# mapillary/OpenSfM

Measured on AMD Instinct MI355X. Metric: image-pairs matched/sec (+ BA LM-iters/sec, 5k cams / 500k pts), higher is better.
Workload: dtype i8 (exact int32 accumulate) + f64 RANSAC

## Files before the change

### opensfm_amd/csrc/ba.hip

```cpp
#ifdef OSFM_HIPEMU
#include <cassert>
#endif
#include <chrono>
#include <cmath>
#include <cstdio>
#include <cstring>
#include <numeric>
#include <vector>

#include <rocprim/rocprim.hpp>

#include "ba_math.h"
#include "osfm_internal.h"

using namespace osfm_ba;

namespace {

constexpr int kCoopObs = 256;

typedef double osfm_v2d __attribute__((ext_vector_type(2)));
__device__ __forceinline__ void st2(double *p, double a, double b) {
  osfm_v2d v;
  v.x = a;
// ... 3248 lines not shown
  for (int t = threadIdx.x; t < n; t += blockDim.x) v[0] += Bc[(long)i * n + t] * z[t];
  block_sum<1, 1024>(v, lds);
  if (threadIdx.x == 0) y[i] = r[cam0 + i] - v[0];
}
__global__ void border_rhs_apply_kernel(const double *SigInv, const double *y, double *z, int nb, int cam0) {
  const int i = blockIdx.x * blockDim.x + threadIdx.x;
  if (i >= nb) return;
  double acc = 0.0;
  for (int j = 0; j < nb; j++) acc += SigInv[i * nb + j] * y[j];
  z[cam0 + i] = acc;
}
__global__ void border_update_kernel(const double *W, double *z, int nb, int n, int cam0) {
  const int t = blockIdx.x * blockDim.x + threadIdx.x;
  if (t >= n) return;
  double acc = 0.0;
  for (int j = 0; j < nb; j++) acc += W[(long)j * n + t] * z[cam0 + j];
  z[t] -= acc;
}


__global__ void border_sigma_kernel(const double *Cm, const double *dots, double *SigInv, int nb, int *status) {
  if (threadIdx.x != 0 || blockIdx.x != 0) return;
  double Sg[36], Inv[36];
  for (int i = 0; i < nb * nb; i++) {
    Sg[i] = Cm[i] - dots[i];
    Inv[i] = 0.0;
  }
  for (int i = 0; i < nb; i++) Inv[i * nb + i] = 1.0;
  int bad = 0;
  for (int c = 0; c < nb && !bad; c++) {
    int piv = c;
    for (int r2 = c + 1; r2 < nb; r2++)
      if (fabs(Sg[r2 * nb + c]) > fabs(Sg[piv * nb + c])) piv = r2;
    const double pv = Sg[piv * nb + c];
    if (!(fabs(pv) > 0) || !(fabs(pv) < 1.0 / 0.0)) { bad = 1; break; }
    for (int q = 0; q < nb; q++) {
      const double t0 = Sg[c * nb + q], t1 = Inv[c * nb + q];
      Sg[c * nb + q] = Sg[piv * nb + q];
      Sg[piv * nb + q] = t0;
      Inv[c * nb + q] = Inv[piv * nb + q];
      Inv[piv * nb + q] = t1;
    }
    const double ip = 1.0 / Sg[c * nb + c];
    for (int q = 0; q < nb; q++) { Sg[c * nb + q] *= ip; Inv[c * nb + q] *= ip; }
    for (int r2 = 0; r2 < nb; r2++) {
      if (r2 == c) continue;
      const double f = Sg[r2 * nb + c];
      for (int q = 0; q < nb; q++) { Sg[r2 * nb + q] -= f * Sg[c * nb + q]; Inv[r2 * nb + q] -= f * Inv[c * nb + q]; }
    }
  }
  *status = bad;
  for (int i = 0; i < nb * nb; i++) SigInv[i] = bad ? 0.0 : Inv[i];
}
template <int NB>
__global__ void __launch_bounds__(kCoopObs) border_point_kernel(Dev d, double *wB) {
  constexpr int NC_ = NB / 3;
  __shared__ double gsum[kCoopObs * 9];
  __shared__ int gcam[kCoopObs];
  __shared__ double vpt[kCoopObs * 3 * NB];
  const int tid = threadIdx.x;
  const int p0 = d.wg_pt[blockIdx.x], p1 = d.wg_pt[blockIdx.x + 1];
  const long o0 = d.pt_off[p0], o1 = d.pt_off[p1];
  const int nobs = (int)(o1 - o0);
  if (nobs <= kCoopObs) {
    double t0[3] = {0, 0, 0}, t1[3] = {0, 0, 0}, jp[6] = {0, 0, 0, 0, 0, 0};
    int pl = 0, cam = 0;
    const long o = o0 + tid;
    if (tid < nobs) {
      pl = d.o_point[o] - p0;
      const int so = d.o_shot[o];
      cam = d.shot_camera[so];
      const double *sck = d.sc_red + d.cam0 + 3 * cam;
      double jk[6];
      row_jk(d, o, so, jk);
#pragma unroll
      for (int k = 0; k < 3; k++) {
        t0[k] = jk[k] * sck[k];
        t1[k] = jk[3 + k] * sck[k];
      }
#pragma unroll
      for (int j = 0; j < 6; j++) jp[j] = JA(o, R_JP + j);
#pragma unroll
      for (int k = 0; k < 3; k++)
#pragma unroll
        for (int j = 0; j < 3; j++) gsum[9 * tid + 3 * k + j] = jp[j] * t0[k] + jp[3 + j] * t1[k];
      gcam[tid] = cam;
    }
    __syncthreads();
    if (tid < p1 - p0) {
      const int p = p0 + tid;
      double u[NB][3];
#pragma unroll
      for (int c = 0; c < NB; c++) u[c][0] = u[c][1] = u[c][2] = 0.0;
      const int a = (int)(d.pt_off[p] - o0), b = (int)(d.pt_off[p + 1] - o0);
      for (int k = a; k < b; k++) {
        const int cc = gcam[k];
#pragma unroll
        for (int c = 0; c < NC_; c++)
          if (c == cc)
#pragma unroll
            for (int q = 0; q < 3; q++)
#pragma unroll
              for (int j = 0; j < 3; j++) u[3 * c + q][j] += gsum[9 * k + 3 * q + j];
      }
      const double *Hh = d.Hhat + 6 * (long)p;
#pragma unroll
      for (int c = 0; c < NB; c++) {
        vpt[(3 * tid + 0) * NB + c] = Hh[0] * u[c][0] + Hh[1] * u[c][1] + Hh[2] * u[c][2];
        vpt[(3 * tid + 1) * NB + c] = Hh[1] * u[c][0] + Hh[3] * u[c][1] + Hh[4] * u[c][2];
        vpt[(3 * tid + 2) * NB + c] = Hh[2] * u[c][0] + Hh[4] * u[c][1] + Hh[5] * u[c][2];
      }
    }
    __syncthreads();
    if (tid < nobs) {
      double2 *dst = reinterpret_cast<double2 *>(wB + 2L * NB * o);
#pragma unroll
      for (int c = 0; c < NB; c++) {
        const double v0 = vpt[(3 * pl + 0) * NB + c], v1 = vpt[(3 * pl + 1) * NB + c], v2 = vpt[(3 * pl + 2) * NB + c];
        const bool own = (c / 3) == cam;
        st2(reinterpret_cast<double *>(dst + c), (own ? t0[c % 3] : 0.0) - (jp[0] * v0 + jp[1] * v1 + jp[2] * v2),
                      (own ? t1[c % 3] : 0.0) - (jp[3] * v0 + jp[4] * v1 + jp[5] * v2));
      }
    }
    return;
  }
  double u[NB][3];
#pragma unroll
  for (int c = 0; c < NB; c++) u[c][0] = u[c][1] = u[c][2] = 0.0;
  for (long o = o0 + tid; o < o1; o += kCoopObs) {
    const int so = d.o_shot[o], cam = d.shot_camera[so];
    const double *sck = d.sc_red + d.cam0 + 3 * cam;
    double jk[6];
    row_jk(d, o, so, jk);
#pragma unroll
    for (int c = 0; c < NC_; c++)
      if (c == cam)
#pragma unroll
        for (int k = 0; k < 3; k++) {
          const double t0 = jk[k] * sck[k], t1 = jk[3 + k] * sck[k];
#pragma unroll
          for (int j = 0; j < 3; j++) u[3 * c + k][j] += JA(o, R_JP + j) * t0 + JA(o, R_JP + 3 + j) * t1;
        }
  }
#pragma unroll
  for (int c = 0; c < NB; c++)
#pragma unroll
    for (int j = 0; j < 3; j++) vpt[(3 * tid + j) * NB + c] = u[c][j];
  __syncthreads();
  for (int h = kCoopObs / 2; h >= 1; h >>= 1) {
    if (tid < h)
      for (int q = 0; q < 3 * NB; q++) vpt[3 * NB * tid + q] += vpt[3 * NB * (tid + h) + q];
    __syncthreads();
  }
  const double *Hh = d.Hhat + 6 * (long)p0;
  double v[NB][3];
#pragma unroll
  for (int c = 0; c < NB; c++) {
    const double u0 = vpt[0 * NB + c], u1 = vpt[1 * NB + c], u2 = vpt[2 * NB + c];
    v[c][0] = Hh[0] * u0 + Hh[1] * u1 + Hh[2] * u2;
    v[c][1] = Hh[1] * u0 + Hh[3] * u1 + Hh[4] * u2;
    v[c][2] = Hh[2] * u0 + Hh[4] * u1 + Hh[5] * u2;
  }
  for (long o = o0 + tid; o < o1; o += kCoopObs) {
    const int so = d.o_shot[o], cam = d.shot_camera[so];
    const double *sck = d.sc_red + d.cam0 + 3 * cam;
    double jk[6];
    row_jk(d, o, so, jk);
#pragma unroll
    for (int c = 0; c < NB; c++) {
      const bool own = (c / 3) == cam;
      const double t0 = own ? jk[c % 3] * sck[c % 3] : 0.0, t1 = own ? jk[3 + c % 3] * sck[c % 3] : 0.0;
      wB[(2L * NB * o) + 2 * c] = t0 - (JA(o, R_JP) * v[c][0] + JA(o, R_JP + 1) * v[c][1] + JA(o, R_JP + 2) * v[c][2]);
      wB[(2L * NB * o) + 2 * c + 1] = t1 - (JA(o, R_JP + 3) * v[c][0] + JA(o, R_JP + 4) * v[c][1] + JA(o, R_JP + 5) * v[c][2]);
    }
  }
}

template <int NB, int W>
__global__ void __launch_bounds__(64 * W) border_shot_kernel(Dev d, const double *wB, double *Bc, double *partB) {
  __shared__ double red[W > 1 ? W * 9 : 1];
  const int s = (int)xcd_contiguous(blockIdx.x, gridDim.x), lane = threadIdx.x;
  double v[NB][9];
#pragma unroll
  for (int c = 0; c < NB; c++)
#pragma unroll
    for (int i = 0; i < 9; i++) v[c][i] = 0.0;
  const ShotFrame f = shot_frame(d, s);
  for (long k = d.shot_off[s] + lane; k < d.shot_off[s + 1]; k += 64 * W) {
    const long o = d.shot_obs[k];
    const double2 *src = reinterpret_cast<const double2 *>(wB + 2L * NB * o);
    double jc0[6], jc1[6], jk0[3], jk1[3];
    {
      double rr[2], jp[6], jc[12], jk[6];
      sm_row(d, f, k, d.sm_wt[k], rr, jp, jc, jk);
#pragma unroll
      for (int j = 0; j < 6; j++) {
        jc0[j] = jc[j];
        jc1[j] = jc[6 + j];
      }
#pragma unroll
      for (int j = 0; j < 3; j++) {
        jk0[j] = jk[j];
        jk1[j] = jk[3 + j];
      }
    }
#pragma unroll
    for (int c = 0; c < NB; c++) {
      const double2 wv = src[c];
#pragma unroll
      for (int j = 0; j < 6; j++) v[c][j] += jc0[j] * wv.x + jc1[j] * wv.y;
#pragma unroll
      for (int j = 0; j < 3; j++) v[c][6 + j] += jk0[j] * wv.x + jk1[j] * wv.y;
    }
  }
#pragma unroll
  for (int c = 0; c < NB; c++) {
    shot_sum<9, W>(v[c], red);
    if (W > 1) __syncthreads();
  }
  if (lane == 0) {
    const long n6 = 6L * d.S;
#pragma unroll
    for (int c = 0; c < NB; c++) {
      for (int j = 0; j < 6; j++) Bc[c * n6 + 6 * s + j] = d.sc_red[6 * s + j] * v[c][j];
      for (int j = 0; j < 3; j++) partB[(long)s * 3 * NB + 3 * c + j] = v[c][6 + j];
    }
  }
}

template <int NB>
__global__ void __launch_bounds__(TPB) border_cam_kernel(Dev d, const double *partB, double *Cm, double radius) {
  __shared__ double lds[4 * 3 * NB];
  const int cam = blockIdx.x;
  double v[3 * NB];
#pragma unroll
  for (int i = 0; i < 3 * NB; i++) v[i] = 0.0;
  for (int s = threadIdx.x; s < d.S; s += TPB)
    if (d.shot_camera[s] == cam)
#pragma unroll
      for (int i = 0; i < 3 * NB; i++) v[i] += partB[(long)s * 3 * NB + i];
  block_sum<3 * NB, TPB>(v, lds);
  if (threadIdx.x == 0)
    for (int c = 0; c < NB; c++)
      for (int k = 0; k < 3; k++) {
        const int i = d.cam0 + 3 * cam + k;
        const bool diag = (3 * cam + k) == c;
        const double y = diag ? d.sc_red[i] : 0.0;
        Cm[(3 * cam + k) * NB + c] = d.sc_red[i] * (v[3 * c + k] + d.prior_diag[i] * y) + (diag ? d.D_red[i] / radius : 0.0);
      }
}

__global__ void iota_int_kernel(int *a, long n) {
  const long i = (long)blockIdx.x * TPB + threadIdx.x;
  if (i < n) a[i] = (int)i;
}
__global__ void gather_byte_kernel(const int *idx, const unsigned char *src, long n, unsigned char *dst) {
  const long i = (long)blockIdx.x * TPB + threadIdx.x;
  if (i < n) dst[i] = src[idx[i]];
}
__global__ void gen_shot_off_kernel(const long *view_off, const int *inst_view0, int S, long *shot_off) {
  const int i = blockIdx.x * TPB + threadIdx.x;
  if (i <= S) shot_off[i] = view_off[inst_view0[i]];
}
__global__ void gather_int_kernel(const int *idx, const int *src, long n, int *dst) {
  const long i = (long)blockIdx.x * TPB + threadIdx.x;
  if (i < n) dst[i] = src[idx[i]];
}
__global__ void lower_bound_kernel(const int *sorted, long n, int nv, long *off) {
  const long v = (long)blockIdx.x * TPB + threadIdx.x;
  if (v > nv) return;
  long lo = 0, hi = n;
  while (lo < hi) {
    const long mid = (lo + hi) >> 1;
    if (sorted[mid] < (int)v)
      lo = mid + 1;
    else
      hi = mid;
  }
  off[v] = lo;
}
// ... 258 lines not shown
      if (e != hipSuccess && want > bytes) {
        (void)hipGetLastError();
        e = ctx ? b->alloc(ctx, bytes) : b->alloc(bytes);
      }
      if (e != hipSuccess) {
        b->p = nullptr;
        delete b;
        return nullptr;
      }
#ifdef OSFM_HIPEMU
      memset(b->p, 0xFF, b->bytes);
#endif
      slabs.push_back(b);
      cur = (char *)b->p;
      left = b->bytes;
      next_slab = std::min(next_slab * 2, (size_t)2 << 30);
    }
    T *p = (T *)cur;
    cur += bytes;
    left -= bytes;
    return p;
  }
  hipStream_t st = nullptr;
  size_t staged = 0;
  static constexpr size_t kStageBytes = (size_t)4 << 20, kStageMax = (size_t)256 << 10;
  template <typename T>
  T *upload(const T *h, size_t n, hipError_t &e) {
    T *p = alloc<T>(n, e);
    if (e != hipSuccess || n == 0) return p;
    const size_t bytes = n * sizeof(T), padded = (bytes + 63) / 64 * 64;
    if (ctx && st && bytes <= kStageMax && staged + padded <= kStageBytes) {
      if (!ctx->h_stage && hipHostMalloc(&ctx->h_stage, kStageBytes, hipHostMallocDefault) != hipSuccess) {
        ctx->h_stage = nullptr;
        (void)hipGetLastError();
      }
      if (ctx->h_stage) {
        char *dst = (char *)ctx->h_stage + staged;
        memcpy(dst, h, bytes);
        staged += padded;
        e = hipMemcpyAsync(p, dst, bytes, hipMemcpyHostToDevice, st);
        return p;
      }
    }
    e = hipMemcpy(p, h, bytes, hipMemcpyHostToDevice);
    return p;
  }
};

inline int nblk(long n, int t = TPB) { return (int)std::max<long>(1, (n + t - 1) / t); }

struct BaSwitches {
  bool no_sband = getenv("OSFM_BA_NO_SBAND") != nullptr;
  bool check_band = getenv("OSFM_BA_CHECK_BAND") != nullptr;
  bool band_per_shot = getenv("OSFM_BA_BAND_PER_SHOT") != nullptr;
  bool wide_ldlt = getenv("OSFM_BA_WIDE_LDLT") != nullptr;
  const char *dense_cr_budget = getenv("OSFM_BA_DENSE_CR_BUDGET");
  bool gen_full_rows = getenv("OSFM_BA_GEN_FULL_ROWS") != nullptr;
  bool no_fast = getenv("OSFM_BA_NO_FAST") != nullptr;
  int fast_fail_at = getenv("OSFM_BA_FAST_FAIL_AT") ? atoi(getenv("OSFM_BA_FAST_FAIL_AT")) : -1;
  bool trace = getenv("OSFM_BA_TRACE") != nullptr;
  bool spin = getenv("OSFM_BA_NO_SPIN") == nullptr;
  double spin_us = getenv("OSFM_BA_SPIN_US") ? atof(getenv("OSFM_BA_SPIN_US")) : 2000.0;
};

int ba_kernel_attributes(int device) {
  static OsfmPerDeviceOnce once;
  return once.run(device, []() -> int {
    constexpr int kWholeLds = 160 * 1024;
    const auto max_lds = [](const void *kernel, int bytes) { return hipFuncSetAttribute(kernel, hipFuncAttributeMaxDynamicSharedMemorySize, bytes); };
    OSFM_HIP(max_lds((const void *)band_assemble_kernel, kWholeLds));
    OSFM_HIP(max_lds((const void *)band_assemble_compact_kernel, kWholeLds));
    OSFM_HIP(max_lds((const void *)band_mfma_kernel<1>, 96 * 1024));
    OSFM_HIP(max_lds((const void *)band_mfma_kernel<2>, 96 * 1024));
    OSFM_HIP(max_lds((const void *)band_mfma_kernel<3>, 96 * 1024));
    OSFM_HIP(max_lds((const void *)band_mfma_kernel<4>, 96 * 1024));
    OSFM_HIP(max_lds((const void *)band_mfma_kernel<5>, 96 * 1024));
    OSFM_HIP(max_lds((const void *)band_mfma_kernel<6>, 96 * 1024));
    for (int q = 2; q <= 10; q++) OSFM_HIP(max_lds((const void *)bcr_level_for(q).fn, kWholeLds));
    OSFM_HIP(max_lds((const void *)sband_factor_kernel, kWholeLds - 256));
    OSFM_HIP(max_lds((const void *)sband_solve_kernel, kWholeLds));
    OSFM_HIP(max_lds((const void *)wide_factor_kernel, kWholeLds));
    OSFM_HIP(max_lds((const void *)dgj_pivot_kernel, kWholeLds));
    OSFM_HIP(max_lds((const void *)band_cholesky_kernel, kWholeLds));
    OSFM_HIP(max_lds((const void *)ctri_inverse_kernel, kWholeLds));
    OSFM_HIP(max_lds((const void *)gen_border_sigma_kernel, kWholeLds - 256));
    return OSFM_OK;
  });
}

typedef void (*band_mfma_fn)(Dev);
inline band_mfma_fn band_mfma_for(int nt) {
  static constexpr band_mfma_fn fn[6] = {band_mfma_kernel<1>, band_mfma_kernel<2>, band_mfma_kernel<3>, band_mfma_kernel<4>, band_mfma_kernel<5>, band_mfma_kernel<6>};
  return fn[nt >= 1 && nt <= 5 ? nt - 1 : 5];
}

struct SolvePlan {
  int nbord = 0;
  int bw_true = 0;
  int track_repeats_shot = 0;
  int *bp_keys = nullptr, *bp_pts = nullptr;
  bool border_ok = true;
  bool all_cams_fixed = false;
  bool wide = false;
  bool dense_cr = false;
  bool win_band = false;
  int win_grid = 0;
// ... 28 lines not shown
  const double rho = cost_change / model_change;
  if (O->verbose & 1)
    fprintf(stderr, "[osfm_ba] it %d cost %.9e -> %.9e rho %.3f radius %.3e pcg %d\n", iter, cost, cost_n, rho, radius, pcg_iterations);
  if (rho > 1e-3) {
    const double t = 2.0 * rho - 1.0;
    radius = radius / std::fmax(1.0 / 3.0, 1.0 - t * t * t);
    radius = std::fmin(1e16, radius);
    decrease_factor = 2.0;
    return LmVerdict::Accepted;
  }
  radius = radius / decrease_factor;
  decrease_factor *= 2.0;
  return LmVerdict::Rejected;
}

struct Solver {
  osfm_ctx *ctx;
  Dev d;
  BaSwitches sw;
  hipStream_t st;
  int loss;
  double loss_a;
  hipStream_t st2 = nullptr;
  hipEvent_t ev_fork = nullptr, ev_join = nullptr;
  int *d_perm = nullptr;
  int *d_status = nullptr;
  double *d_reproj = nullptr;
  double *hscal = nullptr;
  int *hstat = nullptr;
  double *hrr = nullptr;
  int *hseq = nullptr;
  int seq = 0, nbr_ = 0;
  bool spin = false;
  double spin_us = 0.0;
  void *dev_pinned = nullptr;
  int *g_cols = nullptr, *g_col_pos = nullptr;
  int g_ncols = 0;
  double *g_wB = nullptr, *g_vpartB = nullptr;
  int gen_uniform_model = -1;
  bool gen_compact = false;
  bool have_bpri = false;
  std::vector<unsigned char> gen_col_slot;
  bool use_band = false, use_ctri = false, use_bcr = false, use_border = false, use_wide = false;
  bool use_sband = false;
  bool sband_solved = false;
  bool z_solved = false;
  bool joined = true;
  bool have_scale = false;
  double cur_radius = 0.0;
  bool cams_inert = false;
  double *Bc = nullptr, *Wb = nullptr, *SigInv = nullptr, *dots = nullptr;
  double *yb = nullptr;
  static constexpr int kBorderRhsSplit = 6 * 512;
  double *wB = nullptr, *partB = nullptr, *dCm = nullptr;
  double *sbL = nullptr;

  int pinned(int nbr) {
    const size_t need = (size_t)(32 + 2 + nbr + 8) * sizeof(double);
    if (ctx->h_pinned_bytes < need) {
      if (ctx->h_pinned) (void)hipHostFree(ctx->h_pinned);
      ctx->h_pinned = nullptr;
      ctx->h_pinned_bytes = 0;
      OSFM_HIP(hipHostMalloc(&ctx->h_pinned, std::max<size_t>(need, 65536), hipHostMallocDefault));
      ctx->h_pinned_bytes = std::max<size_t>(need, 65536);
    }
    hscal = (double *)ctx->h_pinned;
    hstat = (int *)(hscal + 32);
    hrr = hscal + 34;
    hseq = (int *)(hscal + 34 + nbr);
    nbr_ = nbr;
    for (int i = 0; i < 34; i++) hscal[i] = 0.0;
    *hseq = 0;
    seq = 0;
    spin = sw.spin;
    spin_us = sw.spin_us;
    if (spin) OSFM_HIP(hipHostGetDevicePointer(&dev_pinned, ctx->h_pinned, 0));
    return OSFM_OK;
  }
  int fetch(const double *a, int na, int ha_off, const int *b = nullptr, int nb = 0, int hb_off = 0, const double *c = nullptr, int nc = 0) {
    if (!spin) {
      if (na) OSFM_HIP(hipMemcpyAsync(hscal + ha_off, a, (size_t)na * sizeof(double), hipMemcpyDeviceToHost, st));
      if (nb) OSFM_HIP(hipMemcpyAsync(hstat + hb_off, b, (size_t)nb * sizeof(int), hipMemcpyDeviceToHost, st));
      if (nc) OSFM_HIP(hipMemcpyAsync(hrr, c, (size_t)nc * sizeof(double), hipMemcpyDeviceToHost, st));
      OSFM_HIP(hipStreamSynchronize(st));
      return OSFM_OK;
    }
    double *dh = (double *)dev_pinned;
    const int want = ++seq;
    hipLaunchKernelGGL(publish_kernel, dim3(1), dim3(64), 0, st, a, na, dh + ha_off, b, nb, (int *)(dh + 32) + hb_off, c, nc, dh + 34, (int *)(dh + 34 + nbr_), want);
    OSFM_HIP(hipGetLastError());
    const auto t0 = std::chrono::steady_clock::now();
    for (long it = 0; __atomic_load_n(hseq, __ATOMIC_ACQUIRE) != want; it++) {
      if ((it & 0x3FF) == 0x3FF && std::chrono::duration<double>(std::chrono::steady_clock::now() - t0).count() * 1e6 > spin_us) {
        OSFM_HIP(hipStreamSynchronize(st));
        OSFM_REQUIRE(__atomic_load_n(hseq, __ATOMIC_ACQUIRE) == want, OSFM_E_HIP, "the device never published round trip %d", want);
      }
    }
    return OSFM_OK;
  }

  void rot(const double *poses) { hipLaunchKernelGGL(shot_rot_kernel, dim3(nblk(d.S, 64)), dim3(64), 0, st, d, poses); }

  template <class F>
  void with_gen_model(F &&f) const {
    using std::integral_constant;
    if (d.g.NRr == 3) f(integral_constant<int, 3>{}, integral_constant<int, -1>{});
// ... 352 lines not shown
  void rhs_enqueue(double radius, hipStream_t sq) {
    if (d.gen) {
      gen_rows_apply(1, sq);
      hipLaunchKernelGGL(gen_schur_finish_kernel, dim3(nbr_), dim3(TPB), 0, sq, d, (const double *)d.x, (const double *)d.y, d.b, radius, 1, d.M > 0 ? 1 : 0, 0, (double *)nullptr);
    } else {
      hipLaunchKernelGGL(schur_point_coop_kernel<1>, dim3(d.nwg), dim3(kCoopObs), 0, sq, d, d.y);
      schur_shot(sq);
      hipLaunchKernelGGL(schur_finish_kernel, dim3(matvec_parts()), dim3(TPB), 0, sq, d, (const double *)d.x, (const double *)d.y, d.b, radius, 1, cams_inert ? 1 : 0,
                         (double *)nullptr);
    }
  }
  int fork_side(hipStream_t side2) {
    OSFM_HIP(hipEventRecord(ev_fork, st));
    OSFM_HIP(hipStreamWaitEvent(side2, ev_fork, 0));
    return OSFM_OK;
  }
  int join() {
    if (!joined) OSFM_HIP(hipStreamWaitEvent(st, ev_join, 0));
    joined = true;
    return OSFM_OK;
  }
  int check_band(const SolvePlan &pl, double radius) {
    const size_t nbd = (size_t)d.S * (d.bw + 1) * 36;
    std::vector<double> b_win(nbd), b_shot(nbd);
    OSFM_HIP(hipMemcpyAsync(b_win.data(), d.band, nbd * sizeof(double), hipMemcpyDeviceToHost, st));
    hipLaunchKernelGGL(band_assemble_kernel, dim3(d.S), dim3(TPB), (size_t)(d.bw + 1) * 36 * pl.band_copies * sizeof(double), st, d, radius, pl.band_copies, 0, d.bw + 1);
    OSFM_HIP(hipMemcpyAsync(b_shot.data(), d.band, nbd * sizeof(double), hipMemcpyDeviceToHost, st));
    OSFM_HIP(hipStreamSynchronize(st));
    double amax = 0, dmax = 0;
    for (size_t q = 0; q < nbd; q++) {
      amax = std::max(amax, std::fabs(b_shot[q]));
      dmax = std::max(dmax, std::fabs(b_shot[q] - b_win[q]));
    }
    OSFM_REQUIRE(dmax <= 1e-10 * amax, OSFM_E_NUMERIC, "band_mfma_kernel differs from band_assemble_kernel: max |diff| %.3e against max |entry| %.3e", dmax, amax);
    OSFM_HIP(hipMemcpyAsync(d.band, b_win.data(), nbd * sizeof(double), hipMemcpyHostToDevice, st));
    OSFM_HIP(hipStreamSynchronize(st));
    return OSFM_OK;
  }
  int assemble_band(const SolvePlan &pl, double radius) {
    if (pl.win_band) {
      hipLaunchKernelGGL(band_mfma_for(d.bpNT), dim3(pl.win_grid), dim3(384), pl.win_lds, st, d);
      hipLaunchKernelGGL(band_finish_kernel, dim3(nblk((long)d.S * (d.bw + 1) * 36)), dim3(TPB), 0, st, d, radius);
      if (sw.check_band) OSFM_TRY(check_band(pl, radius));
    } else if (d.bslot) {
      hipLaunchKernelGGL(band_assemble_compact_kernel, dim3(d.S), dim3(TPB), (size_t)pl.bslot_n * 36 * pl.bslot_copies * sizeof(double) + ((d.bw + 1 + 15) / 16) * 16, st, d,
                         radius, pl.bslot_copies, pl.bslot_n);
    } else {
      for (int lo = 0; lo <= d.bw; lo += pl.band_slice)
        hipLaunchKernelGGL(band_assemble_kernel, dim3(d.S), dim3(TPB), (size_t)std::min(pl.band_slice, d.bw + 1 - lo) * 36 * pl.band_copies * sizeof(double), st, d,
                           radius, pl.band_copies, lo, std::min(pl.band_slice, d.bw + 1 - lo));
    }
    return OSFM_OK;
  }
  int side_work(const SolvePlan &pl, double radius, bool fork_here) {
    const hipStream_t sx = pl.side2 ? pl.side2 : st;
    if (pl.side2 && fork_here) OSFM_TRY(fork_side(pl.side2));
    if (pl.want_border && d.gen) {
      gen_border_columns(radius, sx);
    } else if (pl.want_border) {
      if (3 * d.NC == 3) {
        hipLaunchKernelGGL(border_point_kernel<3>, dim3(d.nwg), dim3(kCoopObs), 0, sx, d, wB);
        if (shot_waves() > 1) hipLaunchKernelGGL((border_shot_kernel<3, kShotWavesSmall>), dim3(d.S), dim3(64 * kShotWavesSmall), 0, sx, d, wB, Bc, partB);
        else hipLaunchKernelGGL((border_shot_kernel<3, 1>), dim3(d.S), dim3(64), 0, sx, d, wB, Bc, partB);
        hipLaunchKernelGGL(border_cam_kernel<3>, dim3(d.NC), dim3(TPB), 0, sx, d, partB, dCm, radius);
      } else {
        hipLaunchKernelGGL(border_point_kernel<6>, dim3(d.nwg), dim3(kCoopObs), 0, sx, d, wB);
        if (shot_waves() > 1) hipLaunchKernelGGL((border_shot_kernel<6, kShotWavesSmall>), dim3(d.S), dim3(64 * kShotWavesSmall), 0, sx, d, wB, Bc, partB);
        else hipLaunchKernelGGL((border_shot_kernel<6, 1>), dim3(d.S), dim3(64), 0, sx, d, wB, Bc, partB);
        hipLaunchKernelGGL(border_cam_kernel<6>, dim3(d.NC), dim3(TPB), 0, sx, d, partB, dCm, radius);
      }
    }
    if (!pl.sband_fuse) rhs_enqueue(radius, sx);
    if (pl.side2) OSFM_HIP(hipEventRecord(ev_join, pl.side2));
    return OSFM_OK;
  }
  void border_sigma(int nb, int n6) {
    hipLaunchKernelGGL(border_dots_kernel, dim3(nb * nb), dim3(TPB), 0, st, Bc, Wb, nb, n6, dots);
    if (nb <= 6)
      hipLaunchKernelGGL(border_sigma_kernel, dim3(1), dim3(64), 0, st, dCm, dots, SigInv, nb, d_status + 1);
    else
      hipLaunchKernelGGL(gen_border_sigma_kernel, dim3(1), dim3(256), (size_t)nb * 2 * nb * sizeof(double), st, (const double *)dCm, (const double *)dots, SigInv, nb, d_status + 1);
  }
  int factorise_wide(const SolvePlan &pl) {
    if (pl.dense_cr) {
      OSFM_TRY(dbcr_factor(d_status));
    } else {
      hipLaunchKernelGGL(wide_tiles_kernel, dim3(d.wNB, d.wWb + 1), dim3(256), 0, st, d, d_status);
      const int ntile = d.wWb * (d.wWb + 1) / 2;
      for (int J = 0; J < d.wNB; J++) {
        const int left = std::min(d.wWb, d.wNB - 1 - J);
        hipLaunchKernelGGL(wide_factor_kernel, dim3(1 + (left == d.wWb ? ntile : left * (left + 1) / 2)), dim3(256), (size_t)2 * kWB * kWLd * sizeof(double), st, d, J, d_status);
      }
    }
    use_wide = true;
    if (pl.try_border) {
      const int nb = pl.nbord, n6 = 6 * d.S;
      OSFM_TRY(join());
      wide_solve_set(RhsSet{Bc, n6, Wb, n6, nb + 1, d.b, d.z, nb, d.gen ? -1 : nb});
      z_solved = true;
      border_sigma(nb, n6);
      use_border = true;
    }
    return OSFM_OK;
  }
  int factorise_bcr(const SolvePlan &pl, double radius) {
    const int N = d.ncl;
    if (use_sband) {
      if (pl.fork_in_bcr) OSFM_TRY(side_work(pl, radius, true));
      if (pl.sband_fuse) {
        OSFM_TRY(join());
        hipLaunchKernelGGL(sband_factor_kernel, dim3(1), dim3(kSbThreads), sband_factor_lds(d.S, d.bw), st, d, sbL, d_status, RhsSet{d.b, 0, d.z, 0, 1, nullptr, nullptr, -1, 0},
                           SbFuse{1, radius, d.x, d.r, d.p, d.y, d.scal + 0, d.scal + 4, d.sc_red});
        sband_solved = true;
      } else {
        hipLaunchKernelGGL(sband_factor_kernel, dim3(1), dim3(kSbThreads), sband_factor_lds(d.S, d.bw), st, d, sbL, d_status, RhsSet{nullptr, 0, nullptr, 0, 0, nullptr, nullptr, -1, -1},
                           SbFuse{0, 0.0, nullptr, nullptr, nullptr, nullptr, nullptr, nullptr, nullptr});
      }
    } else {
      hipLaunchKernelGGL(bcr_build_kernel, dim3(N), dim3(256), 0, st, d, d_status);
      const BcrLaunch lv = bcr_level_for(d.cs);
      for (int stq = 1; stq < N; stq *= 2) {
        hipLaunchKernelGGL(lv.fn, dim3((N + 2 * stq - 1) / (2 * stq)), dim3(lv.threads), lv.lds_bytes, st, d, stq, 0, d_status);
        if (stq == 1 && pl.fork_in_bcr) OSFM_TRY(side_work(pl, radius, true));
      }
      hipLaunchKernelGGL(lv.fn, dim3(1), dim3(lv.threads), lv.lds_bytes, st, d, 1, 1, d_status);
// ... 1016 lines not shown
    else free_b += ctx->pool_bytes;
    if (need > free_b - free_b / 8) pl.dense_cr = false;
  }
  if (pl.dense_cr) {
    d.qcs = d.bw;
    d.qm = 6 * d.qcs;
    d.qN = (S + d.qcs - 1) / d.qcs;
    const size_t m2 = (size_t)d.qm * d.qm, nq = (size_t)d.qN;
    d.qD = A.alloc<double>(nq * m2, e);
    d.qE[0] = A.alloc<double>(nq * m2, e);
    d.qE[1] = A.alloc<double>(nq * m2, e);
    d.qX = A.alloc<double>(nq * 2 * m2, e);
    d.qXt = A.alloc<double>(nq * 2 * m2, e);
    d.qx = A.alloc<double>(nq * d.qm * 4, e);
    d.qy = A.alloc<double>(nq * d.qm * 4, e);
    {
      const int np = (d.qm + kWB - 1) / kWB;
      d.qT = ((d.qm + np - 1) / np + 5) / 6 * 6;
      const size_t nb = nq / 2 + 1;
      d.qP = A.alloc<double>(nb * d.qT * d.qT, e);
      d.qR = A.alloc<double>(nb * d.qT * d.qm, e);
      d.qRn = A.alloc<double>(nb * d.qT * d.qm, e);
      d.qC = A.alloc<double>(nb * d.qT * d.qm, e);
    }
  }
  if (pl.wide && !pl.dense_cr) {
    d.wNB = (S + kWcs - 1) / kWcs;
    d.wWb = std::min((d.bw + kWcs - 1) / kWcs, d.wNB - 1);
    const size_t nt = (size_t)d.wNB * (d.wWb + 1) * kWB * kWB;
    d.wA = A.alloc<double>(nt, e);
    d.wL = A.alloc<double>(nt, e);
    d.wLt = A.alloc<double>(nt, e);
    d.wDinv = A.alloc<double>((size_t)d.wNB * kWB * kWB, e);
    d.wx = A.alloc<double>((size_t)d.wNB * kWB * 4, e);
  }
  return OSFM_OK;
}

static int plan_border_and_iteration(const osfm_ba_problem *P, const osfm_ba_options *O, const GenInput *G, Arena &A, hipError_t &e, Solver &sv, SolvePlan &pl) {
  Dev &d = sv.d;
  GenDev &g = d.g;
  const bool gen = G != nullptr;
  const int S = d.S, NC = d.NC;
  const long M = d.M;
  const int nbord = pl.nbord;
  if ((d.ncl > 0 || pl.wide) && nbord >= 1 && nbord <= (gen ? kGenMaxNB : 6)) {
    sv.Bc = A.alloc<double>((size_t)nbord * 6 * S, e);
    sv.Wb = A.alloc<double>((size_t)nbord * 6 * S, e);
    sv.SigInv = A.alloc<double>((size_t)nbord * nbord, e);
    sv.yb = A.alloc<double>((size_t)nbord + 8, e);
    sv.dots = A.alloc<double>((size_t)nbord * nbord, e);
    sv.dCm = A.alloc<double>((size_t)nbord * nbord, e);
    if (!gen) {
      sv.wB = A.alloc<double>((size_t)2 * 3 * NC * M, e);
      sv.partB = A.alloc<double>((size_t)S * 9 * NC, e);
    } else {
      std::vector<int> cols, col_pos((size_t)nbord, -1);
      for (int j = 0; j < nbord; j++) {
        bool held = false;
        for (int v = 0; v < G->NV && !held; v++) held = sv.gen_col_slot[(size_t)j * G->NV + v] != 255;
        if (held) {
          col_pos[(size_t)j] = (int)cols.size();
          cols.push_back(j);
        }
      }
      sv.g_ncols = (int)cols.size();
      if (cols.empty()) cols.push_back(0);
      sv.g_cols = A.upload(cols.data(), cols.size(), e);
      sv.g_col_pos = A.upload(col_pos.data(), col_pos.size(), e);
      sv.g_wB = A.alloc<double>((size_t)std::max<long>(1, M) * std::max(1, sv.g_ncols) * g.NRr, e);
      sv.g_vpartB = A.alloc<double>((size_t)std::max(1, G->NV) * std::max(1, sv.g_ncols) * std::max(1, g.KW), e);
    }
  }
  pl.all_cams_fixed = !gen;
  for (int c = 0; c < NC && !gen; c++) {
    if (P->cam_fixed[c]) pl.border_ok = false;
    else pl.all_cams_fixed = false;
  }
  sv.cams_inert = pl.all_cams_fixed;
  if (pl.all_cams_fixed && e == hipSuccess) OSFM_HIP(hipMemsetAsync(d.camred, 0, (size_t)9 * NC * sizeof(double), sv.st));
  pl.try_bcr = d.bw > 0 && d.ncl > 0 && O->preconditioner == 0;
  pl.try_border = (pl.try_bcr || pl.wide) && sv.Bc && pl.border_ok;
  pl.want_border = d.bw > 0 && (d.ncl > 0 || pl.wide) && O->preconditioner == 0 && sv.Bc && pl.border_ok;
  pl.sband_fuse = sv.use_sband && !gen && pl.all_cams_fixed && d.bw > 0 && d.ncl > 0 && O->preconditioner == 0 && !pl.want_border;
  pl.side2 = pl.sband_fuse ? nullptr : sv.st2;
  pl.fork_at = pl.sband_fuse ? 0 : pl.win_band ? (d.ncl > 1 && O->preconditioner == 0 ? 2 : 1) : 0;
  pl.fork_in_bcr = pl.fork_at == 2 && pl.side2 && d.bw > 0 && d.ncl > 1 && O->preconditioner == 0;
  pl.exact_expected = (pl.try_bcr || pl.wide) && (pl.try_border || (gen ? g.NB == 0 : pl.all_cams_fixed)) && O->pcg_direct_tolerance > O->pcg_tolerance;
  return OSFM_OK;
}

static int write_outputs(osfm_ba_problem *P, const GenInput *G, Arena &A, hipError_t &e, Solver &sv) {
  Dev &d = sv.d;
  GenDev &g = d.g;
  const bool gen = G != nullptr;
  const int S = d.S, NP = d.P, NC = d.NC;
  const long M = d.M;
  hipStream_t st = sv.st;
  int *d_perm = sv.d_perm;
  double *d_reproj = sv.d_reproj;
  sv.rot(d.poses);
  if (gen) {
    hipLaunchKernelGGL(gen_rc_rot_kernel, dim3(nblk(g.NRC, 64)), dim3(64), 0, st, d, (const double *)g.rc);
    if (d_reproj && M > 0) hipLaunchKernelGGL(gen_reproj_kernel, dim3(nblk(M)), dim3(TPB), 0, st, d, d_reproj);
    OSFM_HIP(hipMemcpyAsync(G->cam, g.cam, (size_t)16 * NC * sizeof(double), hipMemcpyDeviceToHost, st));
    OSFM_HIP(hipMemcpyAsync(G->bias, g.bias, (size_t)7 * NC * sizeof(double), hipMemcpyDeviceToHost, st));
    OSFM_HIP(hipMemcpyAsync(G->rc_pose, g.rc, (size_t)6 * g.NRC * sizeof(double), hipMemcpyDeviceToHost, st));
  } else {
// ... 102 lines not shown
```

Measured before the change: 2.748 million.

## Fuse reduced-system RHS into border point/shot passes as an extra column

```diff
diff --git a/opensfm_amd/csrc/ba.hip b/opensfm_amd/csrc/ba.hip
--- a/opensfm_amd/csrc/ba.hip
+++ b/opensfm_amd/csrc/ba.hip
@@ -3324,12 +3324,9 @@
   *status = bad;
   for (int i = 0; i < nb * nb; i++) SigInv[i] = bad ? 0.0 : Inv[i];
 }
-template <int NB>
-__global__ void __launch_bounds__(kCoopObs) border_point_kernel(Dev d, double *wB) {
-  constexpr int NC_ = NB / 3;
-  __shared__ double gsum[kCoopObs * 9];
-  __shared__ int gcam[kCoopObs];
-  __shared__ double vpt[kCoopObs * 3 * NB];
+template <int NB, bool RHS>
+__device__ __forceinline__ void border_point_pass(const Dev &d, double *wB, double *gsum, int *gcam, double *vpt) {
+  constexpr int NC_ = NB / 3, NW = NB + (RHS ? 1 : 0);
   const int tid = threadIdx.x;
   const int p0 = d.wg_pt[blockIdx.x], p1 = d.wg_pt[blockIdx.x + 1];
   const long o0 = d.pt_off[p0], o1 = d.pt_off[p1];
@@ -3382,16 +3379,31 @@
         vpt[(3 * tid + 1) * NB + c] = Hh[1] * u[c][0] + Hh[3] * u[c][1] + Hh[4] * u[c][2];
         vpt[(3 * tid + 2) * NB + c] = Hh[2] * u[c][0] + Hh[4] * u[c][1] + Hh[5] * u[c][2];
       }
+      if (RHS) {
+        const double u0 = -d.g_pt[3 * (long)p], u1 = -d.g_pt[3 * (long)p + 1], u2 = -d.g_pt[3 * (long)p + 2];
+        const double v0 = Hh[0] * u0 + Hh[1] * u1 + Hh[2] * u2;
+        const double v1 = Hh[1] * u0 + Hh[3] * u1 + Hh[4] * u2;
+        const double v2 = Hh[2] * u0 + Hh[4] * u1 + Hh[5] * u2;
+        for (int k = a; k < b; k++) {
+          gsum[9 * k] = v0;
+          gsum[9 * k + 1] = v1;
+          gsum[9 * k + 2] = v2;
+        }
+      }
     }
     __syncthreads();
     if (tid < nobs) {
-      double2 *dst = reinterpret_cast<double2 *>(wB + 2L * NB * o);
+      double2 *dst = reinterpret_cast<double2 *>(wB + 2L * NW * o);
 #pragma unroll
       for (int c = 0; c < NB; c++) {
         const double v0 = vpt[(3 * pl + 0) * NB + c], v1 = vpt[(3 * pl + 1) * NB + c], v2 = vpt[(3 * pl + 2) * NB + c];
         const bool own = (c / 3) == cam;
         st2(reinterpret_cast<double *>(dst + c), (own ? t0[c % 3] : 0.0) - (jp[0] * v0 + jp[1] * v1 + jp[2] * v2),
                       (own ? t1[c % 3] : 0.0) - (jp[3] * v0 + jp[4] * v1 + jp[5] * v2));
+      }
+      if (RHS) {
+        const double v0 = gsum[9 * tid], v1 = gsum[9 * tid + 1], v2 = gsum[9 * tid + 2];
+        st2(reinterpret_cast<double *>(dst + NB), 0.0 - (jp[0] * v0 + jp[1] * v1 + jp[2] * v2), 0.0 - (jp[3] * v0 + jp[4] * v1 + jp[5] * v2));
       }
     }
     return;
@@ -3433,6 +3445,13 @@
     v[c][1] = Hh[1] * u0 + Hh[3] * u1 + Hh[4] * u2;
     v[c][2] = Hh[2] * u0 + Hh[4] * u1 + Hh[5] * u2;
   }
+  double vr0 = 0, vr1 = 0, vr2 = 0;
+  if (RHS) {
+    const double u0 = -d.g_pt[3 * (long)p0], u1 = -d.g_pt[3 * (long)p0 + 1], u2 = -d.g_pt[3 * (long)p0 + 2];
+    vr0 = Hh[0] * u0 + Hh[1] * u1 + Hh[2] * u2;
+    vr1 = Hh[1] * u0 + Hh[3] * u1 + Hh[4] * u2;
+    vr2 = Hh[2] * u0 + Hh[4] * u1 + Hh[5] * u2;
+  }
   for (long o = o0 + tid; o < o1; o += kCoopObs) {
     const int so = d.o_shot[o], cam = d.shot_camera[so];
     const double *sck = d.sc_red + d.cam0 + 3 * cam;
@@ -3442,25 +3461,45 @@
     for (int c = 0; c < NB; c++) {
       const bool own = (c / 3) == cam;
       const double t0 = own ? jk[c % 3] * sck[c % 3] : 0.0, t1 = own ? jk[3 + c % 3] * sck[c % 3] : 0.0;
-      wB[(2L * NB * o) + 2 * c] = t0 - (JA(o, R_JP) * v[c][0] + JA(o, R_JP + 1) * v[c][1] + JA(o, R_JP + 2) * v[c][2]);
-      wB[(2L * NB * o) + 2 * c + 1] = t1 - (JA(o, R_JP + 3) * v[c][0] + JA(o, R_JP + 4) * v[c][1] + JA(o, R_JP + 5) * v[c][2]);
-    }
-  }
-}
-
-template <int NB, int W>
-__global__ void __launch_bounds__(64 * W) border_shot_kernel(Dev d, const double *wB, double *Bc, double *partB) {
-  __shared__ double red[W > 1 ? W * 9 : 1];
+      wB[(2L * NW * o) + 2 * c] = t0 - (JA(o, R_JP) * v[c][0] + JA(o, R_JP + 1) * v[c][1] + JA(o, R_JP + 2) * v[c][2]);
+      wB[(2L * NW * o) + 2 * c + 1] = t1 - (JA(o, R_JP + 3) * v[c][0] + JA(o, R_JP + 4) * v[c][1] + JA(o, R_JP + 5) * v[c][2]);
+    }
+    if (RHS) {
+      const double m0 = JA(o, R_JP) * vr0 + JA(o, R_JP + 1) * vr1 + JA(o, R_JP + 2) * vr2;
+      const double m1 = JA(o, R_JP + 3) * vr0 + JA(o, R_JP + 4) * vr1 + JA(o, R_JP + 5) * vr2;
+      wB[(2L * NW * o) + 2 * NB] = -m0;
+      wB[(2L * NW * o) + 2 * NB + 1] = -m1;
+    }
+  }
+}
+template <int NB>
+__global__ void __launch_bounds__(kCoopObs) border_point_kernel(Dev d, double *wB) {
+  __shared__ double gsum[kCoopObs * 9];
+  __shared__ int gcam[kCoopObs];
+  __shared__ double vpt[kCoopObs * 3 * NB];
+  border_point_pass<NB, false>(d, wB, gsum, gcam, vpt);
+}
+template <int NB>
+__global__ void __launch_bounds__(kCoopObs) side_point_kernel(Dev d, double *wB) {
+  __shared__ double gsum[kCoopObs * 9];
+  __shared__ int gcam[kCoopObs];
+  __shared__ double vpt[kCoopObs * 3 * NB];
+  border_point_pass<NB, true>(d, wB, gsum, gcam, vpt);
+}
+
+template <int NB, int W, bool RHS, int NR>
+__device__ __forceinline__ void border_shot_pass(const Dev &d, const double *wB, double *Bc, double *partB, double (&red)[NR]) {
+  constexpr int NW = NB + (RHS ? 1 : 0);
   const int s = (int)xcd_contiguous(blockIdx.x, gridDim.x), lane = threadIdx.x;
-  double v[NB][9];
-#pragma unroll
-  for (int c = 0; c < NB; c++)
+  double v[NW][9];
+#pragma unroll
+  for (int c = 0; c < NW; c++)
 #pragma unroll
     for (int i = 0; i < 9; i++) v[c][i] = 0.0;
   const ShotFrame f = shot_frame(d, s);
   for (long k = d.shot_off[s] + lane; k < d.shot_off[s + 1]; k += 64 * W) {
     const long o = d.shot_obs[k];
-    const double2 *src = reinterpret_cast<const double2 *>(wB + 2L * NB * o);
+    const double2 *src = reinterpret_cast<const double2 *>(wB + 2L * NW * o);
     double jc0[6], jc1[6], jk0[3], jk1[3];
     {
       double rr[2], jp[6], jc[12], jk[6];
@@ -3477,7 +3516,7 @@
       }
     }
 #pragma unroll
-    for (int c = 0; c < NB; c++) {
+    for (int c = 0; c < NW; c++) {
       const double2 wv = src[c];
 #pragma unroll
       for (int j = 0; j < 6; j++) v[c][j] += jc0[j] * wv.x + jc1[j] * wv.y;
@@ -3486,7 +3525,7 @@
     }
   }
 #pragma unroll
-  for (int c = 0; c < NB; c++) {
+  for (int c = 0; c < NW; c++) {
     shot_sum<9, W>(v[c], red);
     if (W > 1) __syncthreads();
   }
@@ -3497,7 +3536,21 @@
       for (int j = 0; j < 6; j++) Bc[c * n6 + 6 * s + j] = d.sc_red[6 * s + j] * v[c][j];
       for (int j = 0; j < 3; j++) partB[(long)s * 3 * NB + 3 * c + j] = v[c][6 + j];
     }
-  }
+    if (RHS) {
+      for (int j = 0; j < 6; j++) d.zc[6 * s + j] = v[NW - 1][j];
+      for (int j = 0; j < 3; j++) d.part[9 * (long)s + j] = v[NW - 1][6 + j];
+    }
+  }
+}
+template <int NB, int W>
+__global__ void __launch_bounds__(64 * W) border_shot_kernel(Dev d, const double *wB, double *Bc, double *partB) {
+  __shared__ double red[W > 1 ? W * 9 : 1];
+  border_shot_pass<NB, W, false>(d, wB, Bc, partB, red);
+}
+template <int NB, int W>
+__global__ void __launch_bounds__(64 * W) side_shot_kernel(Dev d, const double *wB, double *Bc, double *partB) {
+  __shared__ double red[W > 1 ? W * 9 : 1];
+  border_shot_pass<NB, W, true>(d, wB, Bc, partB, red);
 }
 
 template <int NB>
@@ -3862,6 +3915,7 @@
 struct BaSwitches {
   bool no_sband = getenv("OSFM_BA_NO_SBAND") != nullptr;
   bool check_band = getenv("OSFM_BA_CHECK_BAND") != nullptr;
+  bool check_side = getenv("OSFM_BA_CHECK_SIDE") != nullptr;
   bool band_per_shot = getenv("OSFM_BA_BAND_PER_SHOT") != nullptr;
   bool wide_ldlt = getenv("OSFM_BA_WIDE_LDLT") != nullptr;
   const char *dense_cr_budget = getenv("OSFM_BA_DENSE_CR_BUDGET");
@@ -3996,6 +4050,7 @@
   double *Bc = nullptr, *Wb = nullptr, *SigInv = nullptr, *dots = nullptr;
   double *yb = nullptr;
   static constexpr int kBorderRhsSplit = 6 * 512;
+  double *chk = nullptr;
   double *wB = nullptr, *partB = nullptr, *dCm = nullptr;
   double *sbL = nullptr;
 
@@ -4454,25 +4509,74 @@
     }
     return OSFM_OK;
   }
+  template <int NB>
+  void border_passes(bool fused, double radius, hipStream_t sx, bool cam_rows = true) {
+    const dim3 pg(d.nwg), pb(kCoopObs), sg(d.S), sb(64 * shot_waves());
+    if (fused) {
+      hipLaunchKernelGGL(side_point_kernel<NB>, pg, pb, 0, sx, d, wB);
+      if (shot_waves() > 1) hipLaunchKernelGGL((side_shot_kernel<NB, kShotWavesSmall>), sg, sb, 0, sx, d, wB, Bc, partB);
+      else hipLaunchKernelGGL((side_shot_kernel<NB, 1>), sg, sb, 0, sx, d, wB, Bc, partB);
+    } else {
+      hipLaunchKernelGGL(border_point_kernel<NB>, pg, pb, 0, sx, d, wB);
+      if (shot_waves() > 1) hipLaunchKernelGGL((border_shot_kernel<NB, kShotWavesSmall>), sg, sb, 0, sx, d, wB, Bc, partB);
+      else hipLaunchKernelGGL((border_shot_kernel<NB, 1>), sg, sb, 0, sx, d, wB, Bc, partB);
+    }
+    if (cam_rows) hipLaunchKernelGGL(border_cam_kernel<NB>, dim3(d.NC), dim3(TPB), 0, sx, d, partB, dCm, radius);
+  }
+  int check_side(double radius, hipStream_t sx) {
+    const int nb = 3 * d.NC;
+    const char *name[5] = {"Bc", "partB", "zc", "part", "b"};
+    double **buf[5] = {&Bc, &partB, &d.zc, &d.part, &d.b};
+    const size_t n[5] = {(size_t)nb * 6 * d.S, (size_t)d.S * 3 * nb, (size_t)6 * d.S, (size_t)9 * d.S, (size_t)d.nred};
+    std::vector<double> h[2][5];
+    const auto fetch = [&](std::vector<double> *to) -> int {
+      for (int a = 0; a < 5; a++) {
+        to[a].resize(n[a]);
+        OSFM_HIP(hipMemcpyAsync(to[a].data(), *buf[a], n[a] * sizeof(double), hipMemcpyDeviceToHost, sx));
+      }
+      OSFM_HIP(hipStreamSynchronize(sx));
+      return OSFM_OK;
+    };
+    OSFM_TRY(fetch(h[0]));
+    OSFM_HIP(hipMemcpyAsync(chk + n[0] + n[1] + n[2], d.part, n[3] * sizeof(double), hipMemcpyDeviceToDevice, sx));
+    double *kept[5], *scratch = chk;
+    for (int a = 0; a < 5; a++) {
+      kept[a] = *buf[a];
+      *buf[a] = scratch;
+      scratch += n[a];
+    }
+    if (nb == 3) border_passes<3>(false, radius, sx, false);
+    else border_passes<6>(false, radius, sx, false);
+    rhs_enqueue(radius, sx);
+    const int rc = fetch(h[1]);
+    for (int a = 0; a < 5; a++) *buf[a] = kept[a];
+    if (rc != OSFM_OK) return rc;
+    for (int a = 0; a < 5; a++) {
+      if (n[a] == 0 || memcmp(h[0][a].data(), h[1][a].data(), n[a] * sizeof(double)) == 0) continue;
+      size_t q = 0;
+      while (memcmp(&h[0][a][q], &h[1][a][q], sizeof(double)) == 0) q++;
+      OSFM_REQUIRE(false, OSFM_E_NUMERIC, "the fused side passes differ from the separate kernels: %s[%zu] is %.17g, not %.17g", name[a], q, h[0][a][q], h[1][a][q]);
+    }
+    if (sw.trace) fprintf(stderr, "[osfm_ba trace] side check: %d border columns and the right-hand side equal the separate kernels'\n", nb);
+    return OSFM_OK;
+  }
   int side_work(const SolvePlan &pl, double radius, bool fork_here) {
     const hipStream_t sx = pl.side2 ? pl.side2 : st;
     if (pl.side2 && fork_here) OSFM_TRY(fork_side(pl.side2));
+    const bool fused = pl.want_border && !d.gen && !pl.sband_fuse;
     if (pl.want_border && d.gen) {
       gen_border_columns(radius, sx);
     } else if (pl.want_border) {
-      if (3 * d.NC == 3) {
-        hipLaunchKernelGGL(border_point_kernel<3>, dim3(d.nwg), dim3(kCoopObs), 0, sx, d, wB);
-        if (shot_waves() > 1) hipLaunchKernelGGL((border_shot_kernel<3, kShotWavesSmall>), dim3(d.S), dim3(64 * kShotWavesSmall), 0, sx, d, wB, Bc, partB);
-        else hipLaunchKernelGGL((border_shot_kernel<3, 1>), dim3(d.S), dim3(64), 0, sx, d, wB, Bc, partB);
-        hipLaunchKernelGGL(border_cam_kernel<3>, dim3(d.NC), dim3(TPB), 0, sx, d, partB, dCm, radius);
-      } else {
-        hipLaunchKernelGGL(border_point_kernel<6>, dim3(d.nwg), dim3(kCoopObs), 0, sx, d, wB);
-        if (shot_waves() > 1) hipLaunchKernelGGL((border_shot_kernel<6, kShotWavesSmall>), dim3(d.S), dim3(64 * kShotWavesSmall), 0, sx, d, wB, Bc, partB);
-        else hipLaunchKernelGGL((border_shot_kernel<6, 1>), dim3(d.S), dim3(64), 0, sx, d, wB, Bc, partB);
-        hipLaunchKernelGGL(border_cam_kernel<6>, dim3(d.NC), dim3(TPB), 0, sx, d, partB, dCm, radius);
-      }
-    }
-    if (!pl.sband_fuse) rhs_enqueue(radius, sx);
+      if (3 * d.NC == 3) border_passes<3>(fused, radius, sx);
+      else border_passes<6>(fused, radius, sx);
+    }
+    if (fused) {
+      hipLaunchKernelGGL(schur_finish_kernel, dim3(matvec_parts()), dim3(TPB), 0, sx, d, (const double *)d.x, (const double *)d.y, d.b, radius, 1, cams_inert ? 1 : 0,
+                         (double *)nullptr);
+      if (sw.check_side) OSFM_TRY(check_side(radius, sx));
+    } else if (!pl.sband_fuse) {
+      rhs_enqueue(radius, sx);
+    }
     if (pl.side2) OSFM_HIP(hipEventRecord(ev_join, pl.side2));
     return OSFM_OK;
   }
@@ -5595,8 +5699,9 @@
     sv.dots = A.alloc<double>((size_t)nbord * nbord, e);
     sv.dCm = A.alloc<double>((size_t)nbord * nbord, e);
     if (!gen) {
-      sv.wB = A.alloc<double>((size_t)2 * 3 * NC * M, e);
+      sv.wB = A.alloc<double>((size_t)2 * (3 * NC + 1) * M, e);
       sv.partB = A.alloc<double>((size_t)S * 9 * NC, e);
+      if (sv.sw.check_side) sv.chk = A.alloc<double>((size_t)nbord * 6 * S + (size_t)S * 9 * NC + 6 * S + 9 * S + d.nred, e);
     } else {
       std::vector<int> cols, col_pos((size_t)nbord, -1);
       for (int j = 0; j < nbord; j++) {
```

Result: no change. 2.742 million (-0.2%).
